# embedded-software-laboratory/p-dmpc

Measured on AMD Instinct MI355X. Metric: MPC steps/sec (whole node) + p50 per-step plan latency, N vehicles H=8, higher is better.
Workload: dtype f64

## Files before the change

### p-dmpc_amd/csrc/bulk_search.hpp

```cpp
#include <hip/hip_runtime.h>

#include "search_common.hpp"

#include "frontier_common.hpp"

#define BK_P2 3
#define BK_PER PDMPC_BK_PER
#define BK_FAST_PER 4

namespace {

typedef volatile LDS_AS unsigned long long lds_vu64;

__device__ __forceinline__ unsigned long long wg_scan_excl(unsigned long long v, lds_vu64* wsum, int lane, int wave, int n_waves, unsigned long long& total) {
    unsigned long long inc = v;
#pragma unroll
    for (int o = 1; o < PDMPC_WAVE; o <<= 1) {
        const unsigned long long t = __shfl_up(inc, o);
        inc += lane >= o ? t : 0ull;
    }
    if (lane == PDMPC_WAVE - 1) wsum[wave] = inc;
    __syncthreads();
    unsigned long long off = 0, tot = 0;
    for (int q = 0; q < n_waves; ++q) {
// ... 268 lines not shown
    uint32_t c = inc - loc, b = 0, cu = 0;
    bool f = false;
#pragma unroll
    for (int q = 0; q < 4; ++q) {
        c += hq[q];
        const bool hit = !f && hq[q] != 0u && c >= want;
        b = hit ? (uint32_t)(4 * lane + q) : b;
        cu = hit ? c : cu;
        f = f || hit;
    }
    const unsigned long long m = __ballot(f);
    const int l = m ? (int)__builtin_ctzll(m) : 0;
    const uint32_t bb = lane_u(b, l), cc = lane_u(cu, l);
    bin = m ? bb : 0u;
    cum = m ? cc : 0u;
}

__device__ __forceinline__ void bk_post_store(d2* p, d2 v) {
    __hip_atomic_store((double*)p, (double)v.x, __ATOMIC_RELAXED, __HIP_MEMORY_SCOPE_AGENT);
    __hip_atomic_store((double*)p + 1, (double)v.y, __ATOMIC_RELAXED, __HIP_MEMORY_SCOPE_AGENT);
}
__device__ __forceinline__ d2 bk_post_load(const d2* p) {
    d2 v;
    v.x = __hip_atomic_load((const double*)p, __ATOMIC_RELAXED, __HIP_MEMORY_SCOPE_AGENT);
    v.y = __hip_atomic_load((const double*)p + 1, __ATOMIC_RELAXED, __HIP_MEMORY_SCOPE_AGENT);
    return v;
}
__device__ __forceinline__ void bk_area_store(double* p, double v) { __hip_atomic_store(p, v, __ATOMIC_RELAXED, __HIP_MEMORY_SCOPE_AGENT); }
__device__ __forceinline__ void bk_area_store_u32(int32_t* p, int v) { __hip_atomic_store(p, (int32_t)v, __ATOMIC_RELAXED, __HIP_MEMORY_SCOPE_AGENT); }
__device__ __forceinline__ double bk_area_load(const double* p) { return __hip_atomic_load(p, __ATOMIC_RELAXED, __HIP_MEMORY_SCOPE_AGENT); }
__device__ __forceinline__ int bk_area_load_i32(const int32_t* p) { return (int)__hip_atomic_load(p, __ATOMIC_RELAXED, __HIP_MEMORY_SCOPE_AGENT); }

__device__ __forceinline__ void bk_write_record(const KernelArgs& A, Ctx& X, uint32_t goal, int status, bool dep_timeout, uint32_t n_popped, uint32_t nnodes, bool path_ready,
                                                const lds_u32* ref_ids, bool again, bool counts_only, int lane) {
    const int Hp = X.Hp;
    const DevVehicle* __restrict__ V = X.V;
    pdmpc_vehicle_out* __restrict__ O = X.O;
    lds_u32* l_path = X.l_path;
    const Search& S = X.S;
    if (counts_only) {
        if (goal && ref_ids && lane <= Hp) O->tree_path[lane] = (int32_t)ref_ids[lane];
        if (lane == 0) {
            O->status = dep_timeout ? PDMPC_ERR_HIP : status;
            O->n_expanded = (int32_t)nnodes;
            O->n_popped = (int32_t)n_popped;
        }
        return;
    }
    lds_d2* pshape = (lds_d2*)(X.lsm + PDMPC_LK_PSHAPE);
    lds_u32* pcols = (lds_u32*)(pshape + Hp * PDMPC_VMAX);
    if (again) {
        double* od = (double*)O;
        const int nd = (int)(offsetof(pdmpc_vehicle_out, path_nodes) / 8) + (Hp + 1) * 8;
        const int y0 = (int)(offsetof(pdmpc_vehicle_out, y_predicted) / 8);
        const double qnan = __longlong_as_double(0x7ff8000000000000LL);
        for (int i = lane; i < nd; i += PDMPC_WAVE) od[i] = (i >= y0 && i < y0 + PDMPC_HP_MAX * 3) ? qnan : 0.0;
        asm volatile("s_waitcnt vmcnt(0)" ::: "memory");
    }
    if (goal) {
        if (lane == 0 && !path_ready) {
            uint32_t nd = goal;
            for (int i = Hp; i >= 0; --i) {
                l_path[i] = nd;
                nd = node_parent(S, nd - 1);
            }
        }
        wave_sync();
        if (lane <= Hp) {
            const uint32_t nd = l_path[lane];
            const NodeRec r = node_load(S, nd - 1);
            O->tree_path[lane] = (int32_t)(ref_ids ? ref_ids[lane] : nd);
            double* row = O->path_nodes[lane];
            row[0] = r.x;
            row[1] = r.y;
            row[2] = r.yaw;
            row[3] = (double)NODE_TRIM(r.packed);
            row[4] = r.g;
            row[5] = r.h;
            row[6] = (double)NODE_K(r.packed);
            row[7] = 1.0;
            if (lane >= 1) {
                O->y_predicted[lane - 1][0] = r.x;
                O->y_predicted[lane - 1][1] = r.y;
                O->y_predicted[lane - 1][2] = r.yaw;
                O->predicted_trims[lane - 1] = (int32_t)NODE_TRIM(r.packed);
            }
        }
        for (int idx = lane; idx < Hp * PDMPC_VMAX; idx += PDMPC_WAVE) {
            const int i = idx / PDMPC_VMAX + 1;
            const int v = idx - (i - 1) * PDMPC_VMAX;
            const NodeRec pr = node_load(S, l_path[i - 1] - 1);
            const NodeRec cr = node_load(S, l_path[i] - 1);
            const int m = NODE_MAN(cr.packed);
            const int ncols = NODE_COLS(cr.packed);
            if (v == 0) {
                bk_area_store_u32(&O->shape_cols[i - 1], ncols);
                pcols[i - 1] = (uint32_t)ncols;
            }
            d2 sp = d2{0.0, 0.0};
            if (v < ncols) {
                const d2 a = X.C.g_area[(size_t)m * 3 * PDMPC_VMAX + v];
                sp.x = pr.cs * a.x - pr.sn * a.y + pr.x;
                sp.y = pr.sn * a.x + pr.cs * a.y + pr.y;
                bk_area_store(&O->shapes[i - 1][0][v], sp.x);
                bk_area_store(&O->shapes[i - 1][1][v], sp.y);
            }
            pshape[idx] = sp;
        }
    } else if (V->fb_off[0] >= 0) {
        for (int idx = lane; idx < Hp * PDMPC_VMAX; idx += PDMPC_WAVE) {
            const int k = idx / PDMPC_VMAX;
            const int v = idx - k * PDMPC_VMAX;
            const int a = V->fb_off[k], b = V->fb_off[k + 1];
            const int cols = (b - a < PDMPC_VMAX) ? (b - a) : PDMPC_VMAX;
            if (v == 0) bk_area_store_u32(&O->shape_cols[k], cols);
            if (v < cols) {
                bk_area_store(&O->shapes[k][0][v], A.points[2 * (size_t)(a + v)]);
                bk_area_store(&O->shapes[k][1][v], A.points[2 * (size_t)(a + v) + 1]);
            }
        }
    }
    if (lane == 0) {
        O->status = dep_timeout ? PDMPC_ERR_HIP : status;
        O->n_expanded = (int32_t)nnodes;
        O->n_popped = (int32_t)n_popped;
        O->n_hp = Hp;
    }
}

__device__ __forceinline__ void bk_publish_flag(const KernelArgs& A, int slot, int lane) {
    asm volatile("s_waitcnt vmcnt(0)" ::: "memory");
    wave_sync();
    if (lane == 0) {
        __hip_atomic_store(A.done_flag + slot, A.epoch, __ATOMIC_RELAXED, __HIP_MEMORY_SCOPE_AGENT);
    }
}
// ... 1135 lines not shown
            __syncthreads();
            BK_TICK(tk_pb)
            if (sh[FR_FLAGS] & FRF_BUG) {
                dep_timeout = true;
                status = PDMPC_EXHAUSTED;
                break;
            }
            const uint32_t need = sh[BK_RP_NEED];
            if (need) {
                if (tid == 0) {
                    ready[0] = need;
                    r_flag[0] = 0u;
                }
                Rn = 1;
                __syncthreads();
                continue;
            }
            goal = sh[BK_RP_GOAL];
            if (sh[BK_PUBLISHED] != 0u && goal != best) atomicOr((uint32_t*)&sh[FR_FLAGS], FRF_BUG);
            R.n_popped = sh[BK_RP_NPOP];
            R.n_expanded = sh[BK_RP_NREF];
            pb_valid = true;
            rec_valid = false;
            tie_replayed = true;
            status = goal ? PDMPC_OK : PDMPC_EXHAUSTED;
            __syncthreads();
            if (sh[FR_FLAGS] & FRF_BUG) dep_timeout = true;
            break;
        }
        BK_MARK2
        const bool publish_first = done && !unverified && !pb_valid && sh[BK_PUBLISHED] == 0u && sh_load64(sh, SH_PEND_LO) == 0ull;
        if (done && (unverified || publish_first) && !dep_timeout) {
            if (!rec_valid && sh[BK_PUBLISHED] == 0u) {
                if (wave == 0) bk_write_record(A, X, best, best ? PDMPC_OK : PDMPC_EXHAUSTED, false, R.n_popped, R.n_expanded, false, nullptr, rec_written, false, lane);
                rec_written = true;
            }
            __syncthreads();
            if (wave == 0 && sh[BK_PUBLISHED] == 0u)
                bk_wait_done(A.done_flag, P.pred, P.out, A.epoch, (uint32_t)slot, P.l_soup, P.l_soff, P.l_lit, (lds_d2*)(X.lsm + PDMPC_LK_PSHAPE), sh, Hp, P.n_pred, best != 0u,
                             ticking ? (lds_vu64*)(tk + tk_pub) : (lds_vu64*)nullptr, sh_load64(sh, BK_FD_LO), 0u, CHECKER == PDMPC_CHECK_SAT, lane);
            __syncthreads();
            BK_TICK2(4)
            if (unverified) {
                verify_req = true;
                BK_TICK(tk_arrival)
                continue;
            }
        }
        if (done) {
            if (!pb_valid && !dep_timeout) {
                __syncthreads();
                R = fr_phase_b<NW>(A, X, F, EE, best, ref_ids, (LDS_AS unsigned char*)(X.lsm + PDMPC_LK_CAND), F.near_key, F.near_id, gp_path);
                pb_valid = true;
                BK_TICK(tk_pb)
                const uint32_t pflags = sh[FR_FLAGS];
                __syncthreads();
                if (pflags & FRF_TIE) {
                    pb_valid = false;
                    continue;
                }
                if (pflags & FRF_BUG) dep_timeout = true;
            }
            if (sh_load64(sh, SH_PEND_LO) == 0ull || dep_timeout) {
                goal = best;
                status = best ? PDMPC_OK : PDMPC_EXHAUSTED;
                break;
            }
            if (!rec_valid && !dep_timeout) {
                if (wave == 0) bk_write_record(A, X, best, best ? PDMPC_OK : PDMPC_EXHAUSTED, false, R.n_popped, R.n_expanded, best != 0u, ref_ids, rec_written, sh[BK_PUBLISHED] != 0u, lane);
                rec_valid = true;
                rec_written = true;
            }
            if (!vs_copied) {
                uint32_t nn1 = sh[FR_NNODES];
                nn1 = nn1 < S.max_nodes ? nn1 : S.max_nodes;
                const uint32_t nv = VS.NV < nn1 ? VS.NV : nn1;
                for (uint32_t i = (uint32_t)tid; i < nv; i += (uint32_t)bd) VS.g[i] = VS.l[i];
                vs_copied = true;
            }
            if (A.bk_fast_arrival && !dep_timeout) {
                __syncthreads();
                if (wave == 0)
                    bk_wait_done(A.done_flag, P.pred, P.out, A.epoch, (uint32_t)slot, P.l_soup, P.l_soff, P.l_lit, (lds_d2*)(X.lsm + PDMPC_LK_PSHAPE), sh, Hp, P.n_pred, best != 0u,
                                 ticking ? (lds_vu64*)(tk + tk_pub) : (lds_vu64*)nullptr, 0ull, 4096u, CHECKER == PDMPC_CHECK_SAT, lane);
                __syncthreads();
                if (ticking && sh[BK_WAITRES] == 1u) {
                    X.O->path_nodes[PDMPC_HP_MAX - 2][6] = (double)sh[FR_ROUNDS];
                    X.O->path_nodes[PDMPC_HP_MAX - 2][7] = (double)__builtin_amdgcn_s_memrealtime();
                }
                if (sh[BK_IDLE] > A.spin_limit) dep_timeout = true;
            } else if (bk_wait()) {
                dep_timeout = true;
            }
            BK_TICK(tk_wait)
            continue;
        }

        BK_OPAQUE_TID
        uint32_t round_target;
        {
            const uint32_t done_so_far = sh[FR_PROCESSED];
            const uint32_t depth_now = sh[BK_DEPTH];
// ... 481 lines not shown
                    if (lane == 0)
                        old = __hip_atomic_fetch_add(A.help_board + (size_t)(A.first + best_rel) * PDMPC_HB_WORDS + PDMPC_HB_SEATS, 1ull, __ATOMIC_RELAXED, __HIP_MEMORY_SCOPE_AGENT);
                    const uint32_t lo32 = uni_u((uint32_t)old), hi32 = uni_u((uint32_t)(old >> 32));
                    if (hi32 == A.launch_id && lo32 < (uint32_t)PDMPC_HB_SEATS_MAX) got = lo32;
                }
                uint32_t cmd = 0;
                if (got != 0xffffffffu) {
                    cmd = 1;
                } else {
                    const uint32_t fin = __hip_atomic_load(A.help_finished, __ATOMIC_RELAXED, __HIP_MEMORY_SCOPE_AGENT);
                    if (fin - A.help_fin_base >= (uint32_t)n_s) cmd = 2;
                }
                if (lane == 0) {
                    hs[HS_SLOT] = (uint32_t)(A.first + (best_rel >= 0 ? best_rel : 0));
                    hs[HS_FIRST] = got;
                    hs[HS_CMD] = cmd;
                }
            }
            __syncthreads();
            const uint32_t cmd = hs[HS_CMD];
            if (cmd == 2u) break;
            if (cmd == 0u) {
                __builtin_amdgcn_s_sleep(127);
                __builtin_amdgcn_s_sleep(127);
                if (++idle > (A.spin_limit >> 4)) break;
                __syncthreads();
                continue;
            }
            my_slot = (int)hs[HS_SLOT];
            my_seat = (int)hs[HS_FIRST];
            last_seq = 0;
            idle = 0;
            const DevVehicle* __restrict__ V = A.veh + my_slot;
            const int pred_cols = V->n_pred * PDMPC_VMAX;
            int off = 0;
            for (int k = 0; k < Hp; ++k) {
                const int a = V->lit_off[k], b = V->lit_off[k + 1];
                if (tid == 0) {
                    l_soff[k] = off;
                    l_lit[k] = b - a;
                }
                stage16(l_soup + off, (const d2*)A.points + a, b - a, tid);
                off += (b - a) + pred_cols;
            }
            if (tid == 0) l_soff[Hp] = off;
            for (int k = 0; k < Hp; ++k) {
                const int a = V->hdv_off[k], b = V->hdv_off[k + 1];
                if (tid == 0) l_hoff[k] = off;
                stage16(l_soup + off, (const d2*)A.points + a, b - a, tid);
                off += (b - a);
            }
            if (tid == 0) l_hoff[Hp] = off;
            stage16(l_soup + off, (const d2*)A.points + V->ll_off, V->ll_len, tid);
            CK.ll_base = off;
            CK.ll_len = V->ll_len;
            __syncthreads();
            const d2 nanpt = d2{__longlong_as_double(0x7ff8000000000000LL), __longlong_as_double(0x7ff8000000000000LL)};
            for (int idx = tid; idx < Hp * pred_cols; idx += bd) {
                const int k = idx / pred_cols;
                l_soup[l_soff[k] + l_lit[k] + (idx - k * pred_cols)] = nanpt;
            }
            __syncthreads();
            P.pred = A.pred + V->pred_off;
            P.n_pred = V->n_pred;
            if (A.bk_tentative) bk_tentative_areas(A, P, V->n_pred >= 64 ? ~0ull : ((1ull << V->n_pred) - 1ull), tid, bd);
            cur_mask = 0;
            __syncthreads();
            if (tid < 8) {
                const int ls = tid;
                uint32_t mx = 0;
                for (int k = 1; k <= Hp; ++k) {
                    const int M_k = l_soff[k] - l_soff[k - 1], Hk = l_hoff[k] - l_hoff[k - 1];
                    int n0, n1, n2;
                    bk_item_counts<CHECKER>(M_k, Hk, CK.ll_len, n0, n1, n2);
                    const int Sg = 1 << ls;
                    const uint32_t ch = (uint32_t)(((n0 + Sg - 1) >> ls) + ((n1 + Sg - 1) >> ls) + ((n2 + Sg - 1) >> ls));
                    mx = ch > mx ? ch : mx;
                }
                chm[ls] = mx;
            }
            __syncthreads();
            if (hticking) hk_mark = __builtin_amdgcn_s_memrealtime();
            continue;
        }
        unsigned long long* board = A.help_board + (size_t)my_slot * PDMPC_HB_WORDS;
        if (wave == 0) {
            const unsigned long long w = __hip_atomic_load(board + PDMPC_HB_ASSIGN + my_seat, __ATOMIC_RELAXED, __HIP_MEMORY_SCOPE_AGENT);
            const uint32_t seq = (uint32_t)(w >> 40);
            uint32_t cmd = 0;
            if (seq != last_seq && seq != 0u) {
                cmd = 1;
                const unsigned long long mask = __hip_atomic_load(board + PDMPC_HB_MASK, __ATOMIC_RELAXED, __HIP_MEMORY_SCOPE_AGENT);
                if (lane == 0) {
                    hs[HS_FIRST] = (uint32_t)((w >> 20) & 0xfffffull);
// ... 68 lines not shown
        HK_TICK(4)
        hk_tiles += 1;
    }
    if (hticking) {
        atomicAdd(A.work_count + 7, __builtin_amdgcn_s_memrealtime() - hk_start);
        for (int i = 0; i < 5; ++i) atomicAdd(A.work_count + 8 + i, hk[i]);
        atomicAdd(A.work_count + 13, hk_tiles);
    }
#undef HK_TICK
}

template <int NW, int CHECKER>
__device__ __forceinline__ void bulk_body(const KernelArgs& A) {
    if ((int)blockIdx.x < A.bk_helpers_first || (int)blockIdx.x >= A.bk_helpers_first + A.n_searches) {
        bulk_helper_body<CHECKER>(A);
        return;
    }
    extern __shared__ __attribute__((aligned(16))) unsigned char smem[];
    Ctx X;
    const unsigned long long rt0 = __builtin_amdgcn_s_memrealtime();
    search_prologue(A, X, (LDS_AS unsigned char*)smem);
    X.rt_kernel_start = rt0;
    const int wave = X.wave;
    lds_u32* ref_ids = (lds_u32*)(X.lsm + PDMPC_LK_MISC) + 224;
    const bool tie = bulk_search<NW, CHECKER>(A, X, ref_ids);
    (void)tie;
    __syncthreads();
    if (wave != 0) return;
    {
        int l__ = X.lane;
        asm volatile("" : "+v"(l__));
        X.lane = l__;
    }
    if (!X.rec_valid) bk_write_record(A, X, X.goal, X.status, X.dep_timeout, (uint32_t)X.n_popped, X.nnodes, X.path_ready, ref_ids, X.rec_written, X.published, X.lane);
    bk_publish(A, X, X.status, X.dep_timeout);
    if (X.lane == 0 && A.n_helpers > 0) {
        __hip_atomic_store(A.help_board + (size_t)X.slot * PDMPC_HB_WORDS + PDMPC_HB_WANT, 0ull, __ATOMIC_RELAXED, __HIP_MEMORY_SCOPE_AGENT);
        atomicAdd(A.help_finished, 1u);
    }
}

}

#ifndef PDMPC_BULK_KERNEL_ATTR
#define PDMPC_BULK_KERNEL_ATTR
#endif
#define PDMPC_BULK_KERNEL(NAME, LAUNCHER, NW, CHECKER, MAXWAVES)                                                                                   \
    extern "C" __global__ __launch_bounds__(PDMPC_WAVE * (MAXWAVES)) PDMPC_BULK_KERNEL_ATTR void NAME(const KernelArgs A) { bulk_body<NW, CHECKER>(A); } \
    extern "C" int LAUNCHER(const KernelArgs* args, int count, void* stream, uint32_t* lds_high_water) {                                \
        if (count <= 0) return 0;                                                                                                        \
        typedef void (*kernel_t)(const KernelArgs);                                                                                      \
        kernel_t fn = NAME;                                                                                                              \
         \
        uint32_t& have = lds_high_water[0];                                                                                              \
        if (args->lds.total > have) {                                                                                                    \
            hipError_t e = hipFuncSetAttribute((const void*)fn, hipFuncAttributeMaxDynamicSharedMemorySize, (int)args->lds.total);       \
            if (e != hipSuccess) return (int)e;                                                                                          \
            have = args->lds.total;                                                                                                      \
        }                                                                                                                                \
        hipLaunchKernelGGL(fn, dim3(count + (args->n_helpers > 0 ? args->n_helpers : 0)), dim3(PDMPC_WAVE * args->n_waves), args->lds.total, (hipStream_t)stream, *args); \
        return (int)hipGetLastError();                                                                                                   \
    }
```

### p-dmpc_amd/csrc/frontier_common.hpp

```cpp
#pragma once
#include <type_traits>

#define FR_NNODES 32
#define FR_RD_HEAD 33
#define FR_RD_TAIL 34
#define FR_VLIST_N 35
#define FR_NEAR_N 36
#define FR_FAR_N 37
#define FR_FLAGS 38
#define FR_BEST_ID 40
#define FR_SEL_BIN 41
#define FR_SEL_CUM 42
#define FR_SEL2_BIN 43
#define FR_SEL2_CUM 44
#define FR_ROUNDS 45
#define FR_PROCESSED 60
#define FR_BEST_B1 46
#define FR_NEAR_MIN 48
#define FR_NEAR_MAX 50
#define FR_FAR_MIN 52
#define FR_FAR_MAX 54
#define FR_L_FAR 58
#define FR_PATH_FOR 61
#define FR_EVER_INVAL 63
// ... 411 lines not shown
            const lds_d2* poly = polys + p * PDMPC_VMAX;
            d2 q0 = poly[0];
#pragma unroll 1
            for (int j = 0; j + 1 < PDMPC_VMAX; ++j) {
                const d2 q1 = poly[j + 1];
                hit = hit || interx_segment_n<NP>(pt, ne, q0, q1);
                q0 = q1;
            }
        }
    };
    part(std::integral_constant<int, H + 1>{}, 0, ncols - 1 < H ? ncols - 1 : H);
    if (ncols - 1 > H) part(std::integral_constant<int, PDMPC_VMAX - H>{}, H, ncols - 1 - H);
    return hit;
}

struct PhaseB {
    uint32_t n_popped, n_expanded;
};
#define PB_ALIVE 0x100u
#define PB_ONPATH 0x200u
template <int NW>
__device__ PhaseB fr_phase_b(const KernelArgs& A, Ctx& X, const Frontier& F, const ExpandEnv& EE, uint32_t goal, lds_u32* ref_ids, LDS_AS unsigned char* scratch,
                             double* st_b, uint32_t* st_d, const lds_u32* gp_path) {
    int tid = X.tid;
    asm volatile("" : "+v"(tid));
    const int Hp = X.Hp;
    const Search& S = X.S;
    const VState& VS = X.VS;
    lds_u32* l_path = X.l_path;
    lds_f64* Mp = (lds_f64*)F.hist;
    lds_f64* pk = Mp + (PDMPC_HP_MAX + 1) * (PDMPC_HP_MAX + 2);
    lds_u32* cnt_pop = (lds_u32*)(pk + PDMPC_HP_MAX + 1);
    lds_u32* cnt_ch = cnt_pop + PDMPC_HP_MAX + 2;
    lds_u32* ch_d = (lds_u32*)scratch;
    lds_f64* ch_b = (lds_f64*)(scratch + 4 * (size_t)blockDim.x);
    const int n = EE.n, nw = NW > 0 ? NW : EE.nw;
    lds_u32* pkw = cnt_ch + PDMPC_HP_MAX + 2;
    ch_d[tid] = 0;
    const bool have_path = goal && F.sh[FR_PATH_FOR] == goal;
    if (goal && !have_path && tid == 0) {
        uint32_t nd = goal;
        for (int i = Hp; i >= 0; --i) {
            l_path[i] = nd;
            nd = node_parent(S, nd - 1);
        }
    }
    if (have_path && tid <= Hp) l_path[tid] = gp_path[tid];
    if (tid < PDMPC_HP_MAX + 2) {
        cnt_pop[tid] = 0;
        cnt_ch[tid] = 0;
    }
    __syncthreads();
    if (goal && tid <= Hp) {
        const uint32_t nd = l_path[tid];
        pk[tid] = F.gkey[nd - 1];
        pkw[tid] = ((const uint32_t*)(S.gn + (nd - 1u)))[15];
    }
    __syncthreads();
    if (goal && tid <= Hp) {
        double m = -1.0;
        for (int j = tid + 1; j <= Hp; ++j) {
            m = pk[j] > m ? pk[j] : m;
            Mp[tid * (PDMPC_HP_MAX + 2) + j] = m;
        }
    }
    __syncthreads();
    uint32_t N = F.sh[FR_NNODES];
    N = N < S.max_nodes ? N : S.max_nodes;
    for (uint32_t base = 0; base < N; base += blockDim.x) {
        const uint32_t i = base + (uint32_t)tid;
        const bool in = i < N;
        uint32_t par = 0, pk_ = 0, vst = 0;
        double key = 0.0;
        if (in) {
            const uint64_t u = F.glink[i];
            par = (uint32_t)(u & 0xffffffffull);
            pk_ = (uint32_t)(u >> 32);
            key = F.gkey[i];
            vst = vs_load(VS, i);
        }
        const int depth = NODE_K(pk_);
        bool resolved = !in;
        int guard = 0;
        uint32_t my_d = 0;
        double my_b = -1.0;
        for (;;) {
            if (!resolved) {
                if (!par) {
                    my_d = PB_ALIVE | (goal ? PB_ONPATH : 0u);
                    resolved = true;
                } else {
                    const uint32_t pi = par - 1u;
                    bool have = false;
                    uint32_t pd = 0;
                    double pb = -1.0;
                    if (pi < base) {
                        pd = st_d[pi];
                        pb = st_b[pi];
                        have = true;
                    } else if (ch_d[pi - base] & 0x80000000u) {
                        pd = ch_d[pi - base] & 0x7fffffffu;
                        pb = ch_b[pi - base];
                        have = true;
                    }
                    if (have) {
                        const bool alive = (pd & PB_ALIVE) && vs_load(VS, pi) == VS_VALID;
                        if (!alive) {
                            my_d = 0;
                        } else if (!goal) {
                            my_d = PB_ALIVE;
                        } else if ((pd & PB_ONPATH) && l_path[depth] == i + 1u) {
                            my_d = PB_ALIVE | PB_ONPATH | (uint32_t)depth;
                        } else if (pd & PB_ONPATH) {
                            my_d = PB_ALIVE | (uint32_t)(depth - 1);
                            my_b = key;
                        } else {
                            my_d = PB_ALIVE | (pd & 0xffu);
                            my_b = pb > key ? pb : key;
                        }
                        resolved = true;
                    }
                }
                if (resolved) {
                    ch_b[tid] = my_b;
                    ch_d[tid] = my_d | 0x80000000u;
                }
            }
            {
                const int sw = FR_SLOWEST + (guard & 1);
                if (tid == 0) F.sh[sw] = 1u;
                __syncthreads();
                if (!resolved) F.sh[sw] = 0u;
                __syncthreads();
                if (F.sh[sw] != 0u) break;
            }
            if (++guard > PDMPC_HP_MAX + 4) {
                if (tid == 0) atomicOr((uint32_t*)&F.sh[FR_FLAGS], FRF_BUG);
                break;
            }
        }
        ch_d[tid] = 0;
        if (in) {
            st_d[i] = my_d;
            st_b[i] = my_b;
        }
        if (in && (my_d & PB_ALIVE)) {
            int t;
            if (!goal) {
                t = 0;
            } else if (my_d & PB_ONPATH) {
                t = depth + 1;
            } else {
                const int d = (int)(my_d & 0xffu);
                t = Hp + 1;
                for (int j = d + 1; j <= Hp; ++j) {
                    const double m = Mp[d * (PDMPC_HP_MAX + 2) + j];
                    if (my_b == m) atomicOr((uint32_t*)&F.sh[FR_FLAGS], FRF_TIE);
                    if (my_b < m) {
                        t = j;
                        break;
                    }
                }
            }
            if (t <= Hp) {
                if (vst == VS_UNKNOWN) atomicOr((uint32_t*)&F.sh[FR_FLAGS], FRF_BUG);
                atomicAdd((uint32_t*)&cnt_pop[t], 1u);
                if (vst == VS_VALID && depth < Hp) {
                    const lds_mask64* mrow = EE.l_mask + ((size_t)depth * n + (NODE_TRIM(pk_) - 1)) * nw;
                    uint32_t c = 0;
                    for (int w = 0; w < nw; ++w) c += (uint32_t)__builtin_popcountll(mrow[w]);
                    atomicAdd((uint32_t*)&cnt_ch[t], c);
                }
            }
        }
        __syncthreads();
    }
    __syncthreads();
    PhaseB R;
    R.n_popped = 0;
    R.n_expanded = 1;
    if (!goal) {
        R.n_popped = cnt_pop[0];
        R.n_expanded = 1u + cnt_ch[0];
        return R;
    }
    if (tid == 0) {
        uint32_t s = 1;
        ref_ids[0] = 1;
        for (int j = 0; j < Hp; ++j) {
            s += cnt_ch[j];
            const uint32_t ppk = pkw[j], cpk2 = pkw[j + 1];
            const lds_mask64* mrow = EE.l_mask + ((size_t)NODE_K(ppk) * n + (NODE_TRIM(ppk) - 1)) * nw;
            const int t2 = NODE_TRIM(cpk2) - 1;
            uint32_t rank = 0;
            for (int w = 0; w < nw; ++w) {
                const uint64_t m = mrow[w];
                if (w < t2 / 64) rank += (uint32_t)__builtin_popcountll(m);
                if (w == t2 / 64) rank += (uint32_t)__builtin_popcountll(m & ((1ull << (t2 % 64)) - 1ull));
            }
            ref_ids[j + 1] = s + 1u + rank;
        }
    }
    uint32_t np = 1, ne = 1;
    for (int t = 0; t <= Hp; ++t) {
        np += cnt_pop[t];
        ne += cnt_ch[t];
    }
    R.n_popped = np;
// ... 7 lines not shown
```

### p-dmpc_amd/csrc/search_common.hpp

```cpp
#pragma once
#include "../../include/pdmpc_math.h"
#include "pdmpc_device.h"

#define PROF_MEMBERS

namespace {

#include "wave_primitives.hpp"
#include "search_state.hpp"
#include "heap_queue.hpp"
#include "edge_checks.hpp"

#define VS_UNKNOWN 0u
#define VS_VALID 1u
#define VS_INVALID 2u

struct VState {
    volatile lds_u8* l;
    uint8_t* g;
    uint32_t NV;
};
__device__ __forceinline__ uint32_t vs_load(const VState& v, uint32_t i0) {
    if (i0 < v.NV) return (uint32_t)v.l[i0];
    return (uint32_t)__hip_atomic_load(v.g + i0, __ATOMIC_RELAXED, __HIP_MEMORY_SCOPE_WORKGROUP);
// ... 20 lines not shown
namespace {

__device__ __forceinline__ unsigned long long sh_load64(volatile lds_u32* sh, int lo) {
    return (unsigned long long)sh[lo] | ((unsigned long long)sh[lo + 1] << 32);
}

struct SpecCtx {
    volatile lds_u32* sh;
    lds_d2* l_soup;
    const lds_i32* l_soff;
    const lds_i32* l_lit;
    const pdmpc_vehicle_out* out;
    const int32_t* pred;
    int32_t* counters;
    int n_pred, Hp;
};

__device__ __forceinline__ void incorporate_areas(const SpecCtx& P, unsigned long long arr, int tid) {
    const double qnan = __longlong_as_double(0x7ff8000000000000LL);
    while (arr) {
        const int p = (int)__builtin_ctzll(arr);
        arr &= arr - 1;
        const pdmpc_vehicle_out* PO = P.out + P.pred[p];
        for (int idx = tid; idx < P.Hp * PDMPC_VMAX; idx += (int)blockDim.x) {
            const int k = idx / PDMPC_VMAX;
            const int v = idx - k * PDMPC_VMAX;
            const int cols = PO->shape_cols[k];
            const double sx = PO->shapes[k][0][v], sy = PO->shapes[k][1][v];
            d2 pt;
            pt.x = v < cols ? sx : qnan;
            pt.y = v < cols ? sy : qnan;
            P.l_soup[P.l_soff[k] + P.l_lit[k] + p * PDMPC_VMAX + v] = pt;
        }
    }
}

}

struct Ctx {
    int tid, lane, wave, slot, Hp, n, nw;
    const DevVehicle* V;
    lds_mask64* l_mask;
    lds_i16* l_mi;
    lds_pose* l_pose;
    lds_f64 *l_rx, *l_ry;
    volatile lds_u32* l_shared;
    VState VS;
    lds_f64 *l_dcum, *l_term;
    lds_d2* l_chxy;
    Search S;
    CheckCtx C;
    SpecCtx P;
    pdmpc_vehicle_out* O;
    lds_u32* l_path;
    LDS_AS unsigned char* lsm;
    int status, n_popped;
    uint32_t goal, nnodes;
    bool dep_timeout;
    bool rec_valid = false, rec_written = false;
    bool published = false;
    unsigned long long rt_kernel_start = 0;
    bool path_ready = false;
};

struct ExpandEnv {
    lds_mask64* l_mask;
// ... 39 lines not shown
    S.lkey = nullptr;
    S.lid = nullptr;
    S.NL = (uint32_t)A.NL;
    S.HL = 0;
    S.max_nodes = A.max_nodes;
    S.lane = lane;
    S.pl = make_pop_lane(lane);
    S.heap_len = 0;
    const size_t voff = (size_t)slot * A.max_nodes;
    S.gn = A.arena.nodes + voff;
    S.gkey = A.arena.key + voff;
    S.gid = A.arena.far_id + voff;
    VS.g = A.arena.vstate + voff;

    CheckCtx C;
    C.l_area = (const lds_d2*)(lsm + A.lds.area);
    C.g_area = (const d2*)A.man_area;
    C.l_soup = l_soup;
    C.l_soff = l_soff;
    C.l_hoff = l_hoff;
    C.areas_in_lds = A.areas_in_lds;
    C.Hp = Hp;
    C.checker = A.checker;
    C.sh = (lds_d2*)(lsm + PDMPC_LK_SHAPE) + wave * (2 * PDMPC_VMAX + 1);
    C.tally = (LDS_AS unsigned long long*)(C.sh + 2 * PDMPC_VMAX);
    if (lane == 0) {
        C.tally[0] = 0;
        C.tally[1] = 0;
    }
    C.cand = (lds_u32*)(lsm + PDMPC_LK_CAND) + (size_t)wave * A.cand_cap;

    pdmpc_vehicle_out* __restrict__ O = A.out + slot;

    {
        const int mask_bytes = Hp * n * nw * 8;
        stage16(l_mask, A.succ_mask, (mask_bytes + 15) / 16, tid);
        stage16(l_mi, A.man_index, (n * n * 2 + 15) / 16, tid);
        stage16(l_pose, A.man_pose, A.n_man * 2, tid);
        if (A.areas_in_lds) stage16(lsm + A.lds.area, A.man_area, A.n_man * 3 * PDMPC_VMAX, tid);
    }
    if (tid < Hp) {
        l_rx[tid] = V->ref_x[tid];
        l_ry[tid] = V->ref_y[tid];
        l_dtv[tid] = A.dt * V->v_ref[tid];
    }
    if (tid >= PDMPC_WAVE && tid < PDMPC_WAVE + Hp) {
        const int k_exp = tid - PDMPC_WAVE + 1;
        double d = 0.0;
        for (int it = 1; it <= Hp - k_exp; ++it) {
            d = d + A.dt * V->v_ref[k_exp + it - 1];
            l_dcum[(k_exp - 1) * PDMPC_HP_MAX + (it - 1)] = d;
        }
    }
    if (tid == 0) {
        for (int i = 0; i < SH_WORDS; ++i) l_shared[i] = 0;
    }
    {
        double* od = (double*)O;
        const int nd = (int)(sizeof(pdmpc_vehicle_out) / 8);
        const int y0 = (int)(offsetof(pdmpc_vehicle_out, y_predicted) / 8);
        const double qnan = __longlong_as_double(0x7ff8000000000000LL);
        for (int i = tid; i < nd; i += (int)blockDim.x) od[i] = (i >= y0 && i < y0 + PDMPC_HP_MAX * 3) ? qnan : 0.0;
        asm volatile("s_waitcnt vmcnt(0)" ::: "memory");
    }
    __syncthreads();

    const int n_pred = V->n_pred;
    const int pred_cols = n_pred * PDMPC_VMAX;
    {
        int off = 0;
        for (int k = 0; k < Hp; ++k) {
            const int a = V->lit_off[k], b = V->lit_off[k + 1];
            if (tid == 0) {
                l_soff[k] = off;
                l_lit[k] = b - a;
            }
            stage16(l_soup + off, (const d2*)A.points + a, b - a, tid);
            off += (b - a) + pred_cols;
        }
        if (tid == 0) l_soff[Hp] = off;
        for (int k = 0; k < Hp; ++k) {
            const int a = V->hdv_off[k], b = V->hdv_off[k + 1];
            if (tid == 0) l_hoff[k] = off;
            stage16(l_soup + off, (const d2*)A.points + a, b - a, tid);
            off += (b - a);
        }
        if (tid == 0) l_hoff[Hp] = off;
        stage16(l_soup + off, (const d2*)A.points + V->ll_off, V->ll_len, tid);
        if (tid == 0) l_path[PDMPC_HP_MAX + 1] = (uint32_t)off;
    }
    __syncthreads();
    C.ll_base = uni_i((int)l_path[PDMPC_HP_MAX + 1]);
    C.ll_len = uni_i(V->ll_len);

    SpecCtx P;
    P.sh = l_shared;
    P.l_soup = l_soup;
    P.l_soff = l_soff;
    P.l_lit = l_lit;
    P.out = A.out;
    P.pred = A.pred + V->pred_off;
    P.counters = A.tie_count;
    P.n_pred = n_pred;
    P.Hp = Hp;
    bool dep_timeout = false;
    const bool speculate = A.speculate && n_pred <= 64;
    if (n_pred > 0) {
        const d2 nanpt = d2{__longlong_as_double(0x7ff8000000000000LL), __longlong_as_double(0x7ff8000000000000LL)};
        for (int idx = tid; idx < Hp * pred_cols; idx += (int)blockDim.x) {
            const int k = idx / pred_cols;
            l_soup[l_soff[k] + l_lit[k] + (idx - k * pred_cols)] = nanpt;
        }
        if (!speculate) {
            for (int p = 0; p < n_pred; ++p) {
                uint32_t spins = 0;
                while (__hip_atomic_load(A.done_flag + P.pred[p], __ATOMIC_RELAXED, __HIP_MEMORY_SCOPE_AGENT) != A.epoch) {
                    __builtin_amdgcn_s_sleep(8);
                    if (++spins > A.spin_limit) {
                        dep_timeout = true;
                        break;
                    }
                }
            }
        }
        unsigned long long ready = 0;
        if (wave == 0) {
            bool d = false;
            if (lane < n_pred) d = __hip_atomic_load(A.done_flag + P.pred[lane], __ATOMIC_RELAXED, __HIP_MEMORY_SCOPE_AGENT) == A.epoch;
            ready = __ballot(d);
            if (!speculate) ready = (n_pred >= 64) ? ~0ull : ((1ull << n_pred) - 1ull);
            if (lane == 0) {
                const unsigned long long all = (n_pred >= 64) ? ~0ull : ((1ull << n_pred) - 1ull);
                const unsigned long long pend = speculate ? (all & ~ready) : 0ull;
                l_shared[SH_PEND_LO] = (uint32_t)pend;
                l_shared[SH_PEND_HI] = (uint32_t)(pend >> 32);
                l_shared[SH_ARR_LO] = (uint32_t)ready;
                l_shared[SH_ARR_HI] = (uint32_t)(ready >> 32);
            }
            __builtin_amdgcn_fence(__ATOMIC_ACQUIRE, "agent");
            asm volatile("s_waitcnt vmcnt(0)" ::: "memory");
        }
        __syncthreads();
        if (!speculate) {
            const double qnan = __longlong_as_double(0x7ff8000000000000LL);
            for (int idx = tid; idx < Hp * pred_cols; idx += (int)blockDim.x) {
// ... 52 lines not shown
```

### p-dmpc_amd/csrc/wave_primitives.hpp

```cpp
#pragma once

typedef double d2 __attribute__((ext_vector_type(2)));

__device__ __forceinline__ int uni_i(int v) { return __builtin_amdgcn_readfirstlane(v); }
__device__ __forceinline__ uint32_t uni_u(uint32_t v) { return (uint32_t)__builtin_amdgcn_readfirstlane((int)v); }
__device__ __forceinline__ double uni_d(double v) {
    uint64_t u = (uint64_t)__double_as_longlong(v);
    uint32_t lo = (uint32_t)__builtin_amdgcn_readfirstlane((int)(uint32_t)u);
    uint32_t hi = (uint32_t)__builtin_amdgcn_readfirstlane((int)(uint32_t)(u >> 32));
    return __longlong_as_double((long long)(((uint64_t)hi << 32) | lo));
}
__device__ __forceinline__ double lane_d(double v, int lane_uniform) {
    uint64_t u = (uint64_t)__double_as_longlong(v);
    uint32_t lo = (uint32_t)__builtin_amdgcn_readlane((int)(uint32_t)u, lane_uniform);
    uint32_t hi = (uint32_t)__builtin_amdgcn_readlane((int)(uint32_t)(u >> 32), lane_uniform);
    return __longlong_as_double((long long)(((uint64_t)hi << 32) | lo));
}
__device__ __forceinline__ uint32_t lane_u(uint32_t v, int lane_uniform) { return (uint32_t)__builtin_amdgcn_readlane((int)v, lane_uniform); }
__device__ __forceinline__ bool wave_any(bool p) { return __ballot(p) != 0ull; }
__device__ __forceinline__ bool is_nan(double v) { return v != v; }

#define LDS_AS __attribute__((address_space(3)))
typedef LDS_AS d2 lds_d2;
typedef LDS_AS double lds_f64;
typedef LDS_AS uint32_t lds_u32;
typedef LDS_AS int32_t lds_i32;
typedef LDS_AS int16_t lds_i16;
typedef LDS_AS uint8_t lds_u8;
typedef LDS_AS uint64_t lds_mask64;
typedef LDS_AS DevManPose lds_pose;

__device__ __forceinline__ void stage16(LDS_AS void* dst_lds, const void* src, int count, int tid) {
    lds_d2* d = (lds_d2*)dst_lds;
    const d2* s = (const d2*)src;
    for (int i = tid; i < count; i += (int)blockDim.x) d[i] = s[i];
}

__device__ __forceinline__ void wave_sync() {
    __builtin_amdgcn_fence(__ATOMIC_ACQ_REL, "wavefront");
    __builtin_amdgcn_wave_barrier();
}

__device__ __forceinline__ uint32_t lds_load_u32(const volatile lds_u32* p) { return *p; }
```

Before: 1456.

## Batch LDS staging via segment list, prefetch phase-B chunks, shuffle path records

Replaces the many serial per-segment stage16 calls with a segment table built by one wave and a single batched gather loop that keeps several loads in flight per thread. Phase-B propagation now prefetches the next chunk, skips the iterative resolve loop when no parent lies in the current chunk, and drops a per-chunk barrier. bk_write_record loads path nodes once per lane and passes parent data by wave shuffle instead of re-reading node records, optionally reusing a precomputed path and LDS-resident area table. These cut global-load latency and barrier count in setup and record writing, at the cost of more complex indexing and extra LDS bookkeeping.

New measurement: 1458 (median of 2 runs). No clear change (+0.1%).

```diff
diff --git a/p-dmpc_amd/csrc/bulk_search.hpp b/p-dmpc_amd/csrc/bulk_search.hpp
--- a/p-dmpc_amd/csrc/bulk_search.hpp
+++ b/p-dmpc_amd/csrc/bulk_search.hpp
@@ -324,7 +324,7 @@
 __device__ __forceinline__ int bk_area_load_i32(const int32_t* p) { return (int)__hip_atomic_load(p, __ATOMIC_RELAXED, __HIP_MEMORY_SCOPE_AGENT); }
 
 __device__ __forceinline__ void bk_write_record(const KernelArgs& A, Ctx& X, uint32_t goal, int status, bool dep_timeout, uint32_t n_popped, uint32_t nnodes, bool path_ready,
-                                                const lds_u32* ref_ids, bool again, bool counts_only, int lane) {
+                                                const lds_u32* gp_path, const lds_u32* ref_ids, bool again, bool counts_only, int lane) {
     const int Hp = X.Hp;
     const DevVehicle* __restrict__ V = X.V;
     pdmpc_vehicle_out* __restrict__ O = X.O;
@@ -341,6 +341,26 @@
     }
     lds_d2* pshape = (lds_d2*)(X.lsm + PDMPC_LK_PSHAPE);
     lds_u32* pcols = (lds_u32*)(pshape + Hp * PDMPC_VMAX);
+    NodeRec r;
+    r.x = r.y = r.yaw = r.g = r.cs = r.sn = r.h = 0.0;
+    r.parent = r.packed = 0u;
+    uint32_t my_nd = 0;
+    if (goal) {
+        if (gp_path) {
+            if (lane <= Hp) l_path[lane] = gp_path[lane];
+        } else if (lane == 0 && !path_ready) {
+            uint32_t nd = goal;
+            for (int i = Hp; i >= 0; --i) {
+                l_path[i] = nd;
+                nd = node_parent(S, nd - 1);
+            }
+        }
+        wave_sync();
+        if (lane <= Hp) {
+            my_nd = l_path[lane];
+            r = node_load(S, my_nd - 1);
+        }
+    }
     if (again) {
         double* od = (double*)O;
         const int nd = (int)(offsetof(pdmpc_vehicle_out, path_nodes) / 8) + (Hp + 1) * 8;
@@ -350,18 +370,8 @@
         asm volatile("s_waitcnt vmcnt(0)" ::: "memory");
     }
     if (goal) {
-        if (lane == 0 && !path_ready) {
-            uint32_t nd = goal;
-            for (int i = Hp; i >= 0; --i) {
-                l_path[i] = nd;
-                nd = node_parent(S, nd - 1);
-            }
-        }
-        wave_sync();
         if (lane <= Hp) {
-            const uint32_t nd = l_path[lane];
-            const NodeRec r = node_load(S, nd - 1);
-            O->tree_path[lane] = (int32_t)(ref_ids ? ref_ids[lane] : nd);
+            O->tree_path[lane] = (int32_t)(ref_ids ? ref_ids[lane] : my_nd);
             double* row = O->path_nodes[lane];
             row[0] = r.x;
             row[1] = r.y;
@@ -378,22 +388,27 @@
                 O->predicted_trims[lane - 1] = (int32_t)NODE_TRIM(r.packed);
             }
         }
-        for (int idx = lane; idx < Hp * PDMPC_VMAX; idx += PDMPC_WAVE) {
-            const int i = idx / PDMPC_VMAX + 1;
+        for (int base = 0; base < Hp * PDMPC_VMAX; base += PDMPC_WAVE) {
+            const int idx = base + lane;
+            const bool in = idx < Hp * PDMPC_VMAX;
+            const int i = in ? idx / PDMPC_VMAX + 1 : 1;
             const int v = idx - (i - 1) * PDMPC_VMAX;
-            const NodeRec pr = node_load(S, l_path[i - 1] - 1);
-            const NodeRec cr = node_load(S, l_path[i] - 1);
-            const int m = NODE_MAN(cr.packed);
-            const int ncols = NODE_COLS(cr.packed);
+            const double px = __shfl(r.x, i - 1), py = __shfl(r.y, i - 1), pcs = __shfl(r.cs, i - 1), psn = __shfl(r.sn, i - 1);
+            const uint32_t cpk = (uint32_t)__shfl((int)r.packed, i);
+            if (!in) continue;
+            const int m = NODE_MAN(cpk);
+            const int ncols = NODE_COLS(cpk);
             if (v == 0) {
                 bk_area_store_u32(&O->shape_cols[i - 1], ncols);
                 pcols[i - 1] = (uint32_t)ncols;
             }
             d2 sp = d2{0.0, 0.0};
             if (v < ncols) {
-                const d2 a = X.C.g_area[(size_t)m * 3 * PDMPC_VMAX + v];
-                sp.x = pr.cs * a.x - pr.sn * a.y + pr.x;
-                sp.y = pr.sn * a.x + pr.cs * a.y + pr.y;
+                const size_t ai = (size_t)m * 3 * PDMPC_VMAX + v;
+                const uint32_t aoff = l_path[PDMPC_HP_MAX + 1];
+                const d2 a = aoff ? (d2)((const lds_d2*)(X.lsm + aoff))[ai] : X.C.g_area[ai];
+                sp.x = pcs * a.x - psn * a.y + px;
+                sp.y = psn * a.x + pcs * a.y + py;
                 bk_area_store(&O->shapes[i - 1][0][v], sp.x);
                 bk_area_store(&O->shapes[i - 1][1][v], sp.y);
             }
@@ -1595,7 +1610,8 @@
         const bool publish_first = done && !unverified && !pb_valid && sh[BK_PUBLISHED] == 0u && sh_load64(sh, SH_PEND_LO) == 0ull;
         if (done && (unverified || publish_first) && !dep_timeout) {
             if (!rec_valid && sh[BK_PUBLISHED] == 0u) {
-                if (wave == 0) bk_write_record(A, X, best, best ? PDMPC_OK : PDMPC_EXHAUSTED, false, R.n_popped, R.n_expanded, false, nullptr, rec_written, false, lane);
+                if (wave == 0) bk_write_record(A, X, best, best ? PDMPC_OK : PDMPC_EXHAUSTED, false, R.n_popped, R.n_expanded, false, best && sh[FR_PATH_FOR] == best ? gp_path : (const lds_u32*)nullptr, nullptr,
+                                               rec_written, false, lane);
                 rec_written = true;
             }
             __syncthreads();
@@ -1630,7 +1646,7 @@
                 break;
             }
             if (!rec_valid && !dep_timeout) {
-                if (wave == 0) bk_write_record(A, X, best, best ? PDMPC_OK : PDMPC_EXHAUSTED, false, R.n_popped, R.n_expanded, best != 0u, ref_ids, rec_written, sh[BK_PUBLISHED] != 0u, lane);
+                if (wave == 0) bk_write_record(A, X, best, best ? PDMPC_OK : PDMPC_EXHAUSTED, false, R.n_popped, R.n_expanded, best != 0u, nullptr, ref_ids, rec_written, sh[BK_PUBLISHED] != 0u, lane);
                 rec_valid = true;
                 rec_written = true;
             }
@@ -2178,34 +2194,16 @@
             last_seq = 0;
             idle = 0;
             const DevVehicle* __restrict__ V = A.veh + my_slot;
-            const int pred_cols = V->n_pred * PDMPC_VMAX;
-            int off = 0;
-            for (int k = 0; k < Hp; ++k) {
-                const int a = V->lit_off[k], b = V->lit_off[k + 1];
-                if (tid == 0) {
-                    l_soff[k] = off;
-                    l_lit[k] = b - a;
-                }
-                stage16(l_soup + off, (const d2*)A.points + a, b - a, tid);
-                off += (b - a) + pred_cols;
-            }
-            if (tid == 0) l_soff[Hp] = off;
-            for (int k = 0; k < Hp; ++k) {
-                const int a = V->hdv_off[k], b = V->hdv_off[k + 1];
-                if (tid == 0) l_hoff[k] = off;
-                stage16(l_soup + off, (const d2*)A.points + a, b - a, tid);
-                off += (b - a);
-            }
-            if (tid == 0) l_hoff[Hp] = off;
-            stage16(l_soup + off, (const d2*)A.points + V->ll_off, V->ll_len, tid);
-            CK.ll_base = off;
-            CK.ll_len = V->ll_len;
-            __syncthreads();
-            const d2 nanpt = d2{__longlong_as_double(0x7ff8000000000000LL), __longlong_as_double(0x7ff8000000000000LL)};
-            for (int idx = tid; idx < Hp * pred_cols; idx += bd) {
-                const int k = idx / pred_cols;
-                l_soup[l_soff[k] + l_lit[k] + (idx - k * pred_cols)] = nanpt;
-            }
+            const int pred_cols = V->n_pred * PDMPC_VMAX, ll_len = V->ll_len;
+            const StageList T = stage_list_at((lds_i32*)(lsm + PDMPC_LK_CAND), l_soup, 2 * Hp + 1);
+            int tid_s = tid, lane_s = lane;
+            asm volatile("" : "+v"(tid_s), "+v"(lane_s));
+            if (wave == 0) soup_stage_segments(T, V, A.points, Hp, l_soff, l_hoff, l_lit, lane_s);
+            __syncthreads();
+            stage_segments(T, tid_s, bd);
+            soup_nan_fill(l_soup, l_soff, l_lit, Hp, pred_cols, tid_s, bd);
+            CK.ll_base = l_hoff[Hp];
+            CK.ll_len = ll_len;
             __syncthreads();
             P.pred = A.pred + V->pred_off;
             P.n_pred = V->n_pred;
@@ -2340,7 +2338,7 @@
         asm volatile("" : "+v"(l__));
         X.lane = l__;
     }
-    if (!X.rec_valid) bk_write_record(A, X, X.goal, X.status, X.dep_timeout, (uint32_t)X.n_popped, X.nnodes, X.path_ready, ref_ids, X.rec_written, X.published, X.lane);
+    if (!X.rec_valid) bk_write_record(A, X, X.goal, X.status, X.dep_timeout, (uint32_t)X.n_popped, X.nnodes, X.path_ready, nullptr, ref_ids, X.rec_written, X.published, X.lane);
     bk_publish(A, X, X.status, X.dep_timeout);
     if (X.lane == 0 && A.n_helpers > 0) {
         __hip_atomic_store(A.help_board + (size_t)X.slot * PDMPC_HB_WORDS + PDMPC_HB_WANT, 0ull, __ATOMIC_RELAXED, __HIP_MEMORY_SCOPE_AGENT);
diff --git a/p-dmpc_amd/csrc/frontier_common.hpp b/p-dmpc_amd/csrc/frontier_common.hpp
--- a/p-dmpc_amd/csrc/frontier_common.hpp
+++ b/p-dmpc_amd/csrc/frontier_common.hpp
@@ -467,11 +467,13 @@
     lds_f64* pk = Mp + (PDMPC_HP_MAX + 1) * (PDMPC_HP_MAX + 2);
     lds_u32* cnt_pop = (lds_u32*)(pk + PDMPC_HP_MAX + 1);
     lds_u32* cnt_ch = cnt_pop + PDMPC_HP_MAX + 2;
-    lds_u32* ch_d = (lds_u32*)scratch;
-    lds_f64* ch_b = (lds_f64*)(scratch + 4 * (size_t)blockDim.x);
+    volatile lds_u32* ch_d = (volatile lds_u32*)scratch;
+    volatile lds_f64* ch_b = (volatile lds_f64*)(scratch + 4 * (size_t)blockDim.x);
     const int n = EE.n, nw = NW > 0 ? NW : EE.nw;
     lds_u32* pkw = cnt_ch + PDMPC_HP_MAX + 2;
+    volatile lds_u32* mixw = (volatile lds_u32*)(pkw + PDMPC_HP_MAX + 1);
     ch_d[tid] = 0;
+    if (tid < 3) mixw[tid] = 0u;
     const bool have_path = goal && F.sh[FR_PATH_FOR] == goal;
     if (goal && !have_path && tid == 0) {
         uint32_t nd = goal;
@@ -502,79 +504,101 @@
     __syncthreads();
     uint32_t N = F.sh[FR_NNODES];
     N = N < S.max_nodes ? N : S.max_nodes;
-    for (uint32_t base = 0; base < N; base += blockDim.x) {
-        const uint32_t i = base + (uint32_t)tid;
-        const bool in = i < N;
-        uint32_t par = 0, pk_ = 0, vst = 0;
-        double key = 0.0;
-        if (in) {
+    auto load_chunk = [&](uint32_t base_, uint32_t& par, uint32_t& pk_, double& key, uint32_t& vst) {
+        const uint32_t i = base_ + (uint32_t)tid;
+        par = 0;
+        pk_ = 0;
+        vst = 0;
+        key = 0.0;
+        if (i < N) {
             const uint64_t u = F.glink[i];
             par = (uint32_t)(u & 0xffffffffull);
             pk_ = (uint32_t)(u >> 32);
             key = F.gkey[i];
             vst = vs_load(VS, i);
         }
+    };
+    uint32_t n_par, n_pk, n_vst;
+    double n_key;
+    load_chunk(0u, n_par, n_pk, n_key, n_vst);
+    uint32_t cw = 0;
+    for (uint32_t base = 0; base < N; base += blockDim.x) {
+        const uint32_t i = base + (uint32_t)tid;
+        const bool in = i < N;
+        const uint32_t par = n_par, pk_ = n_pk, vst = n_vst;
+        const double key = n_key;
         const int depth = NODE_K(pk_);
-        bool resolved = !in;
-        int guard = 0;
+        const uint32_t cw_next = cw == 2u ? 0u : cw + 1u;
+        if (wave_any(in && par && par - 1u >= base)) mixw[cw] = 1u;
+        if (tid == 0) mixw[cw_next] = 0u;
+        __syncthreads();
+        const bool mixed = mixw[cw] != 0u;
+        if (base + blockDim.x < N) load_chunk(base + blockDim.x, n_par, n_pk, n_key, n_vst);
         uint32_t my_d = 0;
         double my_b = -1.0;
-        for (;;) {
-            if (!resolved) {
-                if (!par) {
-                    my_d = PB_ALIVE | (goal ? PB_ONPATH : 0u);
+        auto try_resolve = [&]() -> bool {
+            if (!par) {
+                my_d = PB_ALIVE | (goal ? PB_ONPATH : 0u);
+                return true;
+            }
+            const uint32_t pi = par - 1u;
+            uint32_t pd = 0;
+            double pb = -1.0;
+            if (pi < base) {
+                pd = st_d[pi];
+                pb = st_b[pi];
+            } else {
+                const uint32_t cd = ch_d[pi - base];
+                if (!(cd & 0x80000000u)) return false;
+                pd = cd & 0x7fffffffu;
+                pb = ch_b[pi - base];
+            }
+            const bool alive = (pd & PB_ALIVE) && vs_load(VS, pi) == VS_VALID;
+            if (!alive) {
+                my_d = 0;
+            } else if (!goal) {
+                my_d = PB_ALIVE;
+            } else if ((pd & PB_ONPATH) && l_path[depth] == i + 1u) {
+                my_d = PB_ALIVE | PB_ONPATH | (uint32_t)depth;
+            } else if (pd & PB_ONPATH) {
+                my_d = PB_ALIVE | (uint32_t)(depth - 1);
+                my_b = key;
+            } else {
+                my_d = PB_ALIVE | (pd & 0xffu);
+                my_b = pb > key ? pb : key;
+            }
+            return true;
+        };
+        if (!mixed) {
+            if (in) try_resolve();
+        } else {
+            bool resolved = !in;
+            auto announce = [&]() {
+                ch_b[tid] = my_b;
+                ch_d[tid] = my_d | 0x80000000u;
+            };
+            int guard = 0;
+            for (;;) {
+                if (!resolved && try_resolve()) {
                     resolved = true;
-                } else {
-                    const uint32_t pi = par - 1u;
-                    bool have = false;
-                    uint32_t pd = 0;
-                    double pb = -1.0;
-                    if (pi < base) {
-                        pd = st_d[pi];
-                        pb = st_b[pi];
-                        have = true;
-                    } else if (ch_d[pi - base] & 0x80000000u) {
-                        pd = ch_d[pi - base] & 0x7fffffffu;
-                        pb = ch_b[pi - base];
-                        have = true;
-                    }
-                    if (have) {
-                        const bool alive = (pd & PB_ALIVE) && vs_load(VS, pi) == VS_VALID;
-                        if (!alive) {
-                            my_d = 0;
-                        } else if (!goal) {
-                            my_d = PB_ALIVE;
-                        } else if ((pd & PB_ONPATH) && l_path[depth] == i + 1u) {
-                            my_d = PB_ALIVE | PB_ONPATH | (uint32_t)depth;
-                        } else if (pd & PB_ONPATH) {
-                            my_d = PB_ALIVE | (uint32_t)(depth - 1);
-                            my_b = key;
-                        } else {
-                            my_d = PB_ALIVE | (pd & 0xffu);
-                            my_b = pb > key ? pb : key;
-                        }
-                        resolved = true;
-                    }
+                    announce();
                 }
-                if (resolved) {
-                    ch_b[tid] = my_b;
-                    ch_d[tid] = my_d | 0x80000000u;
+                {
+                    const int sw = FR_SLOWEST + (guard & 1);
+                    if (tid == 0) F.sh[sw] = 1u;
+                    __syncthreads();
+                    if (!resolved) F.sh[sw] = 0u;
+                    __syncthreads();
+                    if (F.sh[sw] != 0u) break;
                 }
-            }
-            {
-                const int sw = FR_SLOWEST + (guard & 1);
-                if (tid == 0) F.sh[sw] = 1u;
-                __syncthreads();
-                if (!resolved) F.sh[sw] = 0u;
-                __syncthreads();
-                if (F.sh[sw] != 0u) break;
-            }
-            if (++guard > PDMPC_HP_MAX + 4) {
-                if (tid == 0) atomicOr((uint32_t*)&F.sh[FR_FLAGS], FRF_BUG);
-                break;
-            }
-        }
-        ch_d[tid] = 0;
+                if (++guard > PDMPC_HP_MAX + 4) {
+                    if (tid == 0) atomicOr((uint32_t*)&F.sh[FR_FLAGS], FRF_BUG);
+                    break;
+                }
+            }
+            ch_d[tid] = 0;
+        }
+        cw = cw_next;
         if (in) {
             st_d[i] = my_d;
             st_b[i] = my_b;
@@ -608,7 +632,6 @@
                 }
             }
         }
-        __syncthreads();
     }
     __syncthreads();
     PhaseB R;
diff --git a/p-dmpc_amd/csrc/search_common.hpp b/p-dmpc_amd/csrc/search_common.hpp
--- a/p-dmpc_amd/csrc/search_common.hpp
+++ b/p-dmpc_amd/csrc/search_common.hpp
@@ -76,6 +76,44 @@
             pt.y = v < cols ? sy : qnan;
             P.l_soup[P.l_soff[k] + P.l_lit[k] + p * PDMPC_VMAX + v] = pt;
         }
+    }
+}
+
+__device__ __forceinline__ int soup_stage_segments(const StageList& T, const DevVehicle* __restrict__ V, const double* points, int Hp, lds_i32* l_soff, lds_i32* l_hoff, lds_i32* l_lit, int lane) {
+    const d2* pts = (const d2*)points;
+    const int k = lane < Hp ? lane : Hp;
+    const int la = V->lit_off[k], lb = V->lit_off[k < Hp ? k + 1 : Hp], ha = V->hdv_off[k];
+    const int lit0 = V->lit_off[0], litH = V->lit_off[Hp], hdv0 = V->hdv_off[0], hdvH = V->hdv_off[Hp];
+    const int pred_cols = V->n_pred * PDMPC_VMAX, ll_off = V->ll_off, ll_len = V->ll_len;
+    const int L = litH - lit0, H = hdvH - hdv0;
+    const int hbase = L + Hp * pred_cols;
+    if (lane < Hp) {
+        const int s = la - lit0, d = s + k * pred_cols;
+        T.start[k] = s;
+        T.from[k] = (uint64_t)(uintptr_t)(pts + la);
+        T.to[k] = d;
+        l_soff[k] = d;
+        l_lit[k] = lb - la;
+        T.start[Hp + k] = L + (ha - hdv0);
+        T.from[Hp + k] = (uint64_t)(uintptr_t)(pts + ha);
+        T.to[Hp + k] = hbase + (ha - hdv0);
+        l_hoff[k] = hbase + (ha - hdv0);
+    }
+    if (lane == Hp) {
+        l_soff[Hp] = hbase;
+        l_hoff[Hp] = hbase + H;
+        T.start[2 * Hp] = L + H;
+        T.from[2 * Hp] = (uint64_t)(uintptr_t)(pts + ll_off);
+        T.to[2 * Hp] = hbase + H;
+        T.start[2 * Hp + 1] = L + H + ll_len;
+    }
+    return L + H + ll_len;
+}
+__device__ __forceinline__ void soup_nan_fill(lds_d2* l_soup, const lds_i32* l_soff, const lds_i32* l_lit, int Hp, int pred_cols, int tid, int nthreads) {
+    const d2 nanpt = d2{__longlong_as_double(0x7ff8000000000000LL), __longlong_as_double(0x7ff8000000000000LL)};
+    for (int idx = tid; idx < Hp * pred_cols; idx += nthreads) {
+        const int k = idx / pred_cols;
+        l_soup[l_soff[k] + l_lit[k] + (idx - k * pred_cols)] = nanpt;
     }
 }
 
@@ -181,66 +219,63 @@
 
     pdmpc_vehicle_out* __restrict__ O = A.out + slot;
 
+    const StageList T = stage_list_at((lds_i32*)(lsm + PDMPC_LK_CAND), l_soup, 2 * Hp + 5);
+    const int n_pred = V->n_pred, ll_len = V->ll_len;
+    if (wave == 0) {
+        int at = soup_stage_segments(T, V, A.points, Hp, l_soff, l_hoff, l_lit, lane);
+        if (lane == PDMPC_WAVE - 1) {
+            const int s0 = 2 * Hp + 1;
+            auto seg = [&](int j, const void* src, uint32_t lds_off, int count) {
+                T.from[s0 + j] = (uint64_t)(uintptr_t)src;
+                T.to[s0 + j] = ((int)lds_off - (int)A.lds.soup) / 16;
+                at += count;
+                T.start[s0 + j + 1] = at;
+            };
+            seg(0, A.succ_mask, A.lds.mask, (Hp * n * nw * 8 + 15) / 16);
+            seg(1, A.man_index, A.lds.man_index, (n * n * 2 + 15) / 16);
+            seg(2, A.man_pose, A.lds.pose, A.n_man * 2);
+            seg(3, A.man_area, A.lds.area, A.areas_in_lds ? A.n_man * 3 * PDMPC_VMAX : 0);
+        }
+    }
     {
-        const int mask_bytes = Hp * n * nw * 8;
-        stage16(l_mask, A.succ_mask, (mask_bytes + 15) / 16, tid);
-        stage16(l_mi, A.man_index, (n * n * 2 + 15) / 16, tid);
-        stage16(l_pose, A.man_pose, A.n_man * 2, tid);
-        if (A.areas_in_lds) stage16(lsm + A.lds.area, A.man_area, A.n_man * 3 * PDMPC_VMAX, tid);
-    }
-    if (tid < Hp) {
-        l_rx[tid] = V->ref_x[tid];
-        l_ry[tid] = V->ref_y[tid];
-        l_dtv[tid] = A.dt * V->v_ref[tid];
-    }
-    if (tid >= PDMPC_WAVE && tid < PDMPC_WAVE + Hp) {
-        const int k_exp = tid - PDMPC_WAVE + 1;
-        double d = 0.0;
-        for (int it = 1; it <= Hp - k_exp; ++it) {
-            d = d + A.dt * V->v_ref[k_exp + it - 1];
-            l_dcum[(k_exp - 1) * PDMPC_HP_MAX + (it - 1)] = d;
-        }
-    }
-    if (tid == 0) {
-        for (int i = 0; i < SH_WORDS; ++i) l_shared[i] = 0;
-    }
-    {
+        double rx = 0.0, ry = 0.0, vr = 0.0;
+        if (tid < Hp) {
+            rx = V->ref_x[tid];
+            ry = V->ref_y[tid];
+            vr = V->v_ref[tid];
+        }
         double* od = (double*)O;
         const int nd = (int)(sizeof(pdmpc_vehicle_out) / 8);
         const int y0 = (int)(offsetof(pdmpc_vehicle_out, y_predicted) / 8);
         const double qnan = __longlong_as_double(0x7ff8000000000000LL);
         for (int i = tid; i < nd; i += (int)blockDim.x) od[i] = (i >= y0 && i < y0 + PDMPC_HP_MAX * 3) ? qnan : 0.0;
+        if (tid < Hp) {
+            l_rx[tid] = rx;
+            l_ry[tid] = ry;
+            l_dtv[tid] = A.dt * vr;
+        }
+        if (tid == 0) {
+            for (int i = 0; i < SH_WORDS; ++i) l_shared[i] = 0;
+            l_path[PDMPC_HP_MAX + 1] = A.areas_in_lds ? A.lds.area : 0u;
+        }
         asm volatile("s_waitcnt vmcnt(0)" ::: "memory");
     }
     __syncthreads();
 
-    const int n_pred = V->n_pred;
     const int pred_cols = n_pred * PDMPC_VMAX;
-    {
-        int off = 0;
-        for (int k = 0; k < Hp; ++k) {
-            const int a = V->lit_off[k], b = V->lit_off[k + 1];
-            if (tid == 0) {
-                l_soff[k] = off;
-                l_lit[k] = b - a;
-            }
-            stage16(l_soup + off, (const d2*)A.points + a, b - a, tid);
-            off += (b - a) + pred_cols;
-        }
-        if (tid == 0) l_soff[Hp] = off;
-        for (int k = 0; k < Hp; ++k) {
-            const int a = V->hdv_off[k], b = V->hdv_off[k + 1];
-            if (tid == 0) l_hoff[k] = off;
-            stage16(l_soup + off, (const d2*)A.points + a, b - a, tid);
-            off += (b - a);
-        }
-        if (tid == 0) l_hoff[Hp] = off;
-        stage16(l_soup + off, (const d2*)A.points + V->ll_off, V->ll_len, tid);
-        if (tid == 0) l_path[PDMPC_HP_MAX + 1] = (uint32_t)off;
+    stage_segments(T, tid, (int)blockDim.x);
+    soup_nan_fill(l_soup, l_soff, l_lit, Hp, pred_cols, tid, (int)blockDim.x);
+    if (tid >= PDMPC_WAVE && tid < PDMPC_WAVE + Hp) {
+        const int k_exp = tid - PDMPC_WAVE + 1;
+        double d = 0.0;
+        for (int it = 1; it <= Hp - k_exp; ++it) {
+            d = d + l_dtv[k_exp + it - 1];
+            l_dcum[(k_exp - 1) * PDMPC_HP_MAX + (it - 1)] = d;
+        }
     }
     __syncthreads();
-    C.ll_base = uni_i((int)l_path[PDMPC_HP_MAX + 1]);
-    C.ll_len = uni_i(V->ll_len);
+    C.ll_base = uni_i(l_hoff[Hp]);
+    C.ll_len = uni_i(ll_len);
 
     SpecCtx P;
     P.sh = l_shared;
@@ -255,11 +290,6 @@
     bool dep_timeout = false;
     const bool speculate = A.speculate && n_pred <= 64;
     if (n_pred > 0) {
-        const d2 nanpt = d2{__longlong_as_double(0x7ff8000000000000LL), __longlong_as_double(0x7ff8000000000000LL)};
-        for (int idx = tid; idx < Hp * pred_cols; idx += (int)blockDim.x) {
-            const int k = idx / pred_cols;
-            l_soup[l_soff[k] + l_lit[k] + (idx - k * pred_cols)] = nanpt;
-        }
         if (!speculate) {
             for (int p = 0; p < n_pred; ++p) {
                 uint32_t spins = 0;
diff --git a/p-dmpc_amd/csrc/wave_primitives.hpp b/p-dmpc_amd/csrc/wave_primitives.hpp
--- a/p-dmpc_amd/csrc/wave_primitives.hpp
+++ b/p-dmpc_amd/csrc/wave_primitives.hpp
@@ -36,6 +36,53 @@
     for (int i = tid; i < count; i += (int)blockDim.x) d[i] = s[i];
 }
 
+#define STAGE_BATCH 4
+#define STAGE_SEGS_MAX (2 * PDMPC_HP_MAX + 1 + 4)
+#define STAGE_LIST_WORDS (4 * (STAGE_SEGS_MAX + 3))
+struct StageList {
+    lds_d2* dst;
+    lds_i32* start;
+    lds_i32* to;
+    lds_mask64* from;
+    int nseg;
+};
+__device__ __forceinline__ StageList stage_list_at(lds_i32* words, lds_d2* dst, int nseg) {
+    StageList L;
+    L.dst = dst;
+    L.start = words;
+    L.to = words + (STAGE_SEGS_MAX + 3);
+    L.from = (lds_mask64*)(words + 2 * (STAGE_SEGS_MAX + 3));
+    L.nseg = nseg;
+    return L;
+}
+__device__ __forceinline__ void stage_segments(const StageList& L, int tid, int nthreads) {
+    const int total = L.start[L.nseg];
+    for (int i0 = tid; i0 < total; i0 += STAGE_BATCH * nthreads) {
+        int ic[STAGE_BATCH], g[STAGE_BATCH];
+#pragma unroll
+        for (int u = 0; u < STAGE_BATCH; ++u) {
+            const int i = i0 + u * nthreads;
+            ic[u] = i < total ? i : total - 1;
+            g[u] = 0;
+        }
+        for (int j = 1; j < L.nseg; ++j) {
+            const int sj = L.start[j];
+#pragma unroll
+            for (int u = 0; u < STAGE_BATCH; ++u) g[u] += (ic[u] >= sj) ? 1 : 0;
+        }
+        d2 v[STAGE_BATCH];
+        lds_d2* d[STAGE_BATCH];
+#pragma unroll
+        for (int u = 0; u < STAGE_BATCH; ++u) {
+            const int r = ic[u] - L.start[g[u]];
+            v[u] = ((const d2*)(uintptr_t)L.from[g[u]])[r];
+            d[u] = L.dst + (L.to[g[u]] + r);
+        }
+#pragma unroll
+        for (int u = 0; u < STAGE_BATCH; ++u) *d[u] = v[u];
+    }
+}
+
 __device__ __forceinline__ void wave_sync() {
     __builtin_amdgcn_fence(__ATOMIC_ACQ_REL, "wavefront");
     __builtin_amdgcn_wave_barrier();
```
